# sThalham/PyraPose

Measured on AMD Instinct MI355X. Metric: images/sec 640x480 fwd+bwd (train step: fwd + losses + bwd + clipnorm-Adam), higher is better.
Workload: dtype bf16x3+f16c8

## Files before the change

include/pyrapose_hip.h:

```cpp
#ifndef PYRAPOSE_HIP_H
#define PYRAPOSE_HIP_H

#include <stddef.h>
#include <stdint.h>

#ifdef __cplusplus
extern "C" {
#endif

#define PP_OK 0
#define PP_ERR_ARG (-1)
#define PP_ERR_SHAPE (-2)
#define PP_ERR_ALIGN (-3)
#define PP_ERR_NOCTX (-4)
#define PP_ERR_UNSUPPORTED (-5)
#define PP_ERR_COMM (-6)

#define PP_MAX_SEG 5

typedef struct pp_ctx pp_ctx;

int pp_ctx_create(pp_ctx** out, int device, void* hip_stream);
void pp_ctx_destroy(pp_ctx* ctx);
int pp_ctx_set_stream(pp_ctx* ctx, void* hip_stream);
// ... 165 lines not shown
                             const int* count, float loss_weight, float* loss_sum, float* dlogits);
int pp_orth_smoothl1_fwd_bwd(pp_ctx* ctx, const pp_rowspace* rs, int n_anchor, const float* pred, int ld,
                             const float* y_true, float weight, float sigma, const int* count,
                             float loss_weight, float* loss_sum, float* dpred);

typedef struct {
  long long offset;
  long long count;
  int ld;
  int trainable;
  long long scale_off;
  float l2;
} pp_param_desc;

typedef struct pp_optimizer pp_optimizer;
int pp_optimizer_create(pp_ctx* ctx, pp_optimizer** out, const pp_param_desc* descs_host, int n_desc,
                        long long total);
void pp_optimizer_destroy(pp_optimizer* opt);
int pp_grad_global_norm(pp_ctx* ctx, pp_optimizer* opt, const float* w_master, const float* g_eff,
                        const float* scales, float* gnorm_sq, float* l2_loss);
int pp_adam_step_clipnorm(pp_ctx* ctx, pp_optimizer* opt, float* w_master, float* w_eff, const float* g_eff,
                          const float* scales, float* m, float* v, const float* gnorm_sq, float lr,
                          float beta1, float beta2, float eps, float clipnorm, long long step);

int pp_generate_base_anchors_host(int base_size, const float* ratios_host, int n_ratios,
                                  const float* scales_host, int n_scales, double* out_host);
int pp_anchors_shift_f64(pp_ctx* ctx, int n_levels, const int* feat_h_host, const int* feat_w_host,
                         const int* strides_host, int n_anchor, const double* base_anchors_host,
                         double* anchors_out);
int pp_anchors_shift_f32(pp_ctx* ctx, int n_levels, const int* feat_h_host, const int* feat_w_host,
                         const int* strides_host, int n_anchor, const double* base_anchors_host,
                         float* anchors_out);
int pp_compute_overlap_f64(pp_ctx* ctx, int n, const double* boxes, int k, const double* query, double* overlaps);
int pp_compute_gt_annotations(pp_ctx* ctx, int n, const double* anchors, int k, const double* gt_boxes,
                              double negative_overlap, double positive_overlap, int* argmax, signed char* state);

int pp_anchor_targets(pp_ctx* ctx, int n_anchor_total, const double* anchors, int batch,
                      const int* gt_offset_host, const double* gt_boxes, const int* gt_labels,
                      const double* gt_box3d, const int* gt_mask_ids, const unsigned char* id_masks,
                      int mask_h, int mask_w, const int* mask_hw_host, const int* image_hw_host, int num_classes,
                      double negative_overlap, double positive_overlap, int out_mh, int out_mw,
                      float* regression, float* labels, float* mask);
int pp_project_box3d_host(const double* pose7_host, const double* box8x3_host, const double* cam4_host,
                          double* out16_host);
int pp_pil_nearest_index_host(int n_in, int n_out, int* out_host);

// ... 196 lines not shown
```

pyrapose_amd/_lib.py:

```python
import ctypes as C
import os

_HERE = os.path.dirname(os.path.abspath(__file__))
LIB_PATH = os.path.join(_HERE, os.environ.get("PP_LIB") or "libpyrapose_hip.so")

PP_MAX_SEG = 5


class RowSpace(C.Structure):
    _fields_ = [("n_img", C.c_int), ("n_seg", C.c_int), ("h", C.c_int * PP_MAX_SEG), ("w", C.c_int * PP_MAX_SEG)]

    @classmethod
    def make(cls, n_img, shapes):
        rs = cls()
        rs.n_img = int(n_img)
        rs.n_seg = len(shapes)
        for i, (h, w) in enumerate(shapes):
            rs.h[i] = int(h)
            rs.w[i] = int(w)
        return rs

    def rows(self):
        return sum(self.n_img * self.h[i] * self.w[i] for i in range(self.n_seg))

    def shapes(self):
        return [(self.h[i], self.w[i]) for i in range(self.n_seg)]


class ConvDesc(C.Structure):
    _fields_ = [("in_", RowSpace), ("out", RowSpace), ("cin", C.c_int), ("cout", C.c_int), ("kh", C.c_int),
                ("kw", C.c_int), ("stride", C.c_int), ("pad_t", C.c_int), ("pad_l", C.c_int), ("ld_x", C.c_int),
                ("ld_y", C.c_int), ("ld_w", C.c_int)]


class ParamDesc(C.Structure):
    _fields_ = [("offset", C.c_longlong), ("count", C.c_longlong), ("ld", C.c_int), ("trainable", C.c_int),
                ("scale_off", C.c_longlong), ("l2", C.c_float)]


class SplitJob(C.Structure):
    _fields_ = [("w", C.c_void_p), ("fwd_hi", C.c_void_p), ("fwd_lo", C.c_void_p), ("dg_hi", C.c_void_p), ("dg_lo", C.c_void_p),
                ("taps", C.c_int), ("cin", C.c_int), ("cout", C.c_int), ("ld_w", C.c_int), ("tile_begin", C.c_int), ("reserved", C.c_int)]


class TView(C.Structure):
    _fields_ = [("f32", C.c_void_p), ("hi", C.c_void_p), ("lo", C.c_void_p)]


class ConvOpts(C.Structure):
    _fields_ = [("capture_hi", C.c_void_p), ("capture_lo", C.c_void_p), ("add_hi", C.c_void_p), ("add_lo", C.c_void_p),
                ("mask_hi", C.c_void_p), ("skip_flags", C.c_void_p), ("skip_list", C.c_void_p), ("out_flags", C.c_void_p),
                ("out_list", C.c_void_p), ("lazy_out", C.c_int), ("lazy_in", C.c_int)]


def _load():
    if not os.path.exists(LIB_PATH):
        raise ImportError(
            "pyrapose_amd: %s not found. Build it with `python -c 'import __graft_entry__ as g; g.build()'` "
            "or `make -C pyrapose_amd/csrc`. There is no CPU fallback." % LIB_PATH)
    try:
        return C.CDLL(LIB_PATH)
    except OSError as e:
        raise ImportError("pyrapose_amd: cannot load %s: %s" % (LIB_PATH, e))


# ... 54 lines not shown
    "pp_conv2d_nhwc_bwd_data_bf16x3": (_i, [_p, C.POINTER(ConvDesc), _p, _p, _p, _p, _p, _p, _i, _p, _i, _p, _p, _p, C.POINTER(ConvOpts)]),
    "pp_conv2d_nhwc_bwd_data_s2_bf16x3": (_i, [_p, C.POINTER(ConvDesc), _p, _p, _p, _p, _p, _p, _i, _p, _i, _p, _p, _p, C.POINTER(ConvOpts)]),
    "pp_conv_s2_merged": (_i, []),
    "pp_conv2d_nhwc_bwd_weight_bf16x3": (_i, [_p, C.POINTER(ConvDesc), _p, _p, _p, _p, _p, _p, _p, _p, C.POINTER(ConvOpts)]),
    "pp_conv_plan_text": (_i, [C.POINTER(ConvDesc), _i, C.c_uint, _i, _i, _sz, C.c_char_p, _i]),
    "pp_maxpool3x3s2_fwd": (_i, [_p, _i, _i, _i, _i, _p, _i, _i, _p]),
    "pp_upsample_nearest_add_fwd": (_i, [_p, _i, _i, _i, _i, _i, _i, _p, _p, _p]),
    "pp_upsample_nearest_add_bwd": (_i, [_p, _i, _i, _i, _i, _i, _i, _p, _p, _p]),
    "pp_add_n": (_i, [_p, _sz, _p, _p, _p, _p]),
    "pp_relu_fwd": (_i, [_p, C.c_size_t, _p, _p]),
    "pp_preprocess_caffe_u8": (_i, [_p, _i, _i, _i, C.POINTER(C.c_int), _p, _p]),
    "pp_preprocess_caffe_u8_padded": (_i, [_p, _i, _i, _i, _i, _i, _i, C.POINTER(C.c_int), _p, _p]),
    "pp_pack_rgb_to_4_padded": (_i, [_p, _i, _i, _i, _i, _i, _i, _p, _p]),
    "pp_stem7x7s2_fwd_bf16x3": (_i, [_p, _i, _i, _i, _i, _i, _p, _p, _p, _i, _p, _i, _p, _i]),
    "pp_pack_rgb_to_4": (_i, [_p, _sz, _p, _p]),
    "pp_export_head": (_i, [_p, C.POINTER(RowSpace), _i, _i, _p, _i, _i, _p]),
    "pp_count_positives": (_i, [_p, _sz, _p, _sz, _i, _p, _sz, _i, _p, _p]),
    "pp_sigmoid_focal_fwd_bwd": (_i, [_p, C.POINTER(RowSpace), _i, _i, _p, _i, _p, _f, _f, _p, _f, _p, _p]),
    "pp_orth_smoothl1_fwd_bwd": (_i, [_p, C.POINTER(RowSpace), _i, _p, _i, _p, _f, _f, _p, _f, _p, _p]),
    "pp_optimizer_create": (_i, [_p, C.POINTER(_p), C.POINTER(ParamDesc), _i, _ll]),
    "pp_optimizer_destroy": (None, [_p]),
    "pp_grad_global_norm": (_i, [_p, _p, _p, _p, _p, _p, _p]),
    "pp_adam_step_clipnorm": (_i, [_p, _p, _p, _p, _p, _p, _p, _p, _p, _f, _f, _f, _f, _f, _ll]),
    "pp_generate_base_anchors_host": (_i, [_i, C.POINTER(_f), _i, C.POINTER(_f), _i, C.POINTER(_d)]),
    "pp_anchors_shift_f64": (_i, [_p, _i, C.POINTER(_i), C.POINTER(_i), C.POINTER(_i), _i, C.POINTER(_d), _p]),
    "pp_anchors_shift_f32": (_i, [_p, _i, C.POINTER(_i), C.POINTER(_i), C.POINTER(_i), _i, C.POINTER(_d), _p]),
    "pp_compute_overlap_f64": (_i, [_p, _i, _p, _i, _p, _p]),
    "pp_compute_gt_annotations": (_i, [_p, _i, _p, _i, _p, _d, _d, _p, _p]),
    "pp_anchor_targets": (_i, [_p, _i, _p, _i, C.POINTER(_i), _p, _p, _p, _p, _p, _i, _i, C.POINTER(_i), C.POINTER(_i), _i, _d, _d,
                               _i, _i, _p, _p, _p]),
    "pp_project_box3d_host": (_i, [C.POINTER(_d), C.POINTER(_d), C.POINTER(_d), C.POINTER(_d)]),
    "pp_pil_nearest_index_host": (_i, [_i, _i, C.POINTER(_i)]),
    "pp_box3d_decode": (_i, [_p, _i, _i, _p, _p, _p]),
    "pp_score_threshold_compact": (_i, [_p, _i, _i, _i, _p, _f, _i, _p, _p]),
    "pp_filter_workspace_bytes": (_sz, [_i, _i, _i]),
    "pp_pose_error_workspace_bytes": (_sz, [_i, _i]),
    "pp_filter_detections": (_i, [_p, _i, _i, _p, _p, _p, _f, _f, _i, _p, _p, _p, _p, _p]),
    "pp_pose_add_f64": (_i, [_p, _i, _i, _p, _p, _p, _p, _p, _p, _p]),
    "pp_pose_adi_f64": (_i, [_p, _i, _i, _p, _p, _p, _p, _p, _p, _p]),
    "pp_filter_detections_batch": (_i, [_p, _i, _i, _i, _p, _p, _p, _f, _f, _i, _p, _p, _p, _p, _p]),
    "pp_render_workspace_bytes": (_sz, [_i, _i, _i, _i, _i]),
    "pp_render_depth_f32": (_i, [_p, _i, _i, _p, _i, _p, _p, _p, _p, _i, _i, _d, _d, _p, _sz, _p]),
    "pp_render_rgbd_workspace_bytes": (_sz, [_i, _i, _i, _i, _i]),
    "pp_render_rgbd": (_i, [_p, _i, _i, _p, _p, _p, _i, _p, _p, _p, _p, _i, _i, _d, _d, _i, _d, C.POINTER(_d), C.POINTER(_d), _p, _sz,
                            _p, _p, _p, _p]),
    "pp_render_rgbd_tex_workspace_bytes": (_sz, [_i, _i, _i, _i, _i, _i, _i]),
# ... 79 lines not shown
```

pyrapose_amd/csrc/conv3.hip:

```cpp
#include "conv_common.h"
#include "conv4.h"

#define PP_CAT_(a, b) a##b
#define PP_CAT(a, b) PP_CAT_(a, b)
#if PP_FMT == 1
#define PP_API(name) PP_CAT(name, _fmt1)
#else
#define PP_API(name) PP_CAT(name, _fmt0)
#endif
namespace {
#include "planes_fmt.h"

#include "conv3_shared.h"

#ifndef PP_EPI_GF
#define PP_EPI_GF 4
#endif

template <int TM, int TN, bool AP, bool OP>
__global__ __launch_bounds__(256, (TM * TN >= 8) ? 2 : ((TM * TN == 4) ? 3 : 4)) void igemm3_kernel(
    const IgemmParams p, const float* __restrict__ g_src, const uint4* __restrict__ g_ahi, const uint4* __restrict__ g_alo,
    const uint4* __restrict__ g_whi, const uint4* __restrict__ g_wlo,
    const float* __restrict__ g_bias, const float* __restrict__ g_addend, const float* __restrict__ g_mask,
    float* __restrict__ g_out, uint2* __restrict__ g_ohi, uint2* __restrict__ g_olo, int w_rows, int w_ld8) {
// ... 1047 lines not shown
  int lo = 0, hi = n_jobs - 1;
  while (lo < hi) {
    const int mid = (lo + hi + 1) >> 1;
    if (jobs[mid].tile_begin <= (int)blockIdx.x) lo = mid; else hi = mid - 1;
  }
  const pp_split_job j = jobs[lo];
  const int dg_ld = (j.cout + 31) / 32 * 32;
  const int tiles_co = dg_ld / 32, tiles_ci = j.cin / 32;
  int t = (int)blockIdx.x - j.tile_begin;
  const int co_t = t % tiles_co;
  t /= tiles_co;
  const int ci_t = t % tiles_ci, tap = t / tiles_ci;
  split_weights_tile(tap, ci_t * 32, co_t * 32, j.cin, j.cout, j.ld_w, j.w, (unsigned short*)j.fwd_hi, (unsigned short*)j.fwd_lo, j.cout,
                     (unsigned short*)j.dg_hi, (unsigned short*)j.dg_lo, dg_ld);
}

}
extern "C" int PP_API(pp_conv_split_weights_bf16x3_batch)(pp_ctx* ctx, int n_jobs, const pp_split_job* jobs_dev, int total_tiles) {
  PP_REQUIRE_CTX(ctx);
  PP_CHECK_ARG(ctx, n_jobs >= 0 && total_tiles >= 0 && (n_jobs == 0 || jobs_dev), PP_ERR_ARG, "pp_conv_split_weights_bf16x3_batch: bad arguments");
  if (n_jobs == 0 || total_tiles == 0) return PP_OK;
  hipLaunchKernelGGL(split_weights_batch_kernel, dim3((unsigned)total_tiles), dim3(32, 8), 0, ctx->stream, n_jobs, jobs_dev);
  PP_CHECK_LAUNCH(ctx, "pp_conv_split_weights_bf16x3_batch");
  return PP_OK;
}
namespace {

}
extern "C" int PP_API(pp_conv_split_weights_bf16x3)(pp_ctx* ctx, const pp_conv_desc* d, const float* w, void* fwd_hi, void* fwd_lo,
                                            void* dg_hi, void* dg_lo) {
  PP_REQUIRE_CTX(ctx);
  int rc = check_desc(ctx, d, "pp_conv_split_weights_bf16x3");
  if (rc) return rc;
  PP_CHECK_ARG(ctx, w && ((fwd_hi && fwd_lo) || (dg_hi && dg_lo)), PP_ERR_ARG, "pp_conv_split_weights_bf16x3: null tensor");
  PP_CHECK_ARG(ctx, d->cin % 32 == 0, PP_ERR_SHAPE, "pp_conv_split_weights_bf16x3: cin %d must be a multiple of 32", d->cin);
  const int taps = d->kh * d->kw;
  const int dg_ld = (d->cout + 31) / 32 * 32;
  dim3 grid((unsigned)((dg_ld + 31) / 32), (unsigned)((d->cin + 31) / 32), (unsigned)taps);
  hipLaunchKernelGGL(split_weights_kernel, grid, dim3(32, 8), 0, ctx->stream, taps, d->cin, d->cout, d->ld_w, w,
                     (unsigned short*)fwd_hi, (unsigned short*)fwd_lo, d->cout, (unsigned short*)dg_hi, (unsigned short*)dg_lo, dg_ld);
  PP_CHECK_LAUNCH(ctx, "pp_conv_split_weights_bf16x3");
  return PP_OK;
}
namespace {

__global__ void rl_dilate_kernel(const IgemmParams p, const unsigned char* __restrict__ in_flags, unsigned char* __restrict__ out_flags,
// ... 1041 lines not shown
```

pyrapose_amd/csrc/optim.hip:

```cpp
#include <math.h>
#include <stdlib.h>

#include "pp_internal.h"

#define PP_OPT_CHUNK 1024

struct pp_optimizer {
  pp_param_desc* d_descs;
  int2* d_map;
  double* d_partial;
  double* d_partial_l2;
  int n_desc;
  int n_blocks;
  long long total;
};

extern "C" int pp_optimizer_create(pp_ctx* ctx, pp_optimizer** out, const pp_param_desc* descs, int n_desc, long long total) {
  PP_REQUIRE_CTX(ctx);
  PP_CHECK_ARG(ctx, out && descs && n_desc > 0 && total > 0, PP_ERR_ARG, "pp_optimizer_create: bad argument");
  long long n_blocks = 0;
  for (int i = 0; i < n_desc; ++i) {
    PP_CHECK_ARG(ctx, descs[i].offset >= 0 && descs[i].count > 0 && descs[i].offset + descs[i].count <= total && descs[i].ld > 0 &&
                          descs[i].offset % 4 == 0,
                 PP_ERR_SHAPE, "pp_optimizer_create: tensor %d out of range", i);
    n_blocks += (descs[i].count + PP_OPT_CHUNK - 1) / PP_OPT_CHUNK;
  }
  PP_CHECK_ARG(ctx, n_blocks < (1ll << 30), PP_ERR_SHAPE, "pp_optimizer_create: too many chunks");
  pp_optimizer* o = (pp_optimizer*)calloc(1, sizeof(pp_optimizer));
  if (!o) return pp_fail(ctx, PP_ERR_ARG, "pp_optimizer_create: out of host memory");
  o->n_desc = n_desc;
  o->n_blocks = (int)n_blocks;
  o->total = total;
  int2* map = (int2*)malloc(sizeof(int2) * (size_t)n_blocks);
  long long b = 0;
  for (int i = 0; i < n_desc; ++i) {
    long long nc = (descs[i].count + PP_OPT_CHUNK - 1) / PP_OPT_CHUNK;
    for (long long c = 0; c < nc; ++c) map[b++] = make_int2(i, (int)c);
  }
  hipError_t e = hipMalloc((void**)&o->d_descs, sizeof(pp_param_desc) * n_desc);
  if (e == hipSuccess) e = hipMalloc((void**)&o->d_map, sizeof(int2) * (size_t)n_blocks);
  if (e == hipSuccess) e = hipMalloc((void**)&o->d_partial, sizeof(double) * (size_t)n_blocks);
  if (e == hipSuccess) e = hipMalloc((void**)&o->d_partial_l2, sizeof(double) * (size_t)n_blocks);
  if (e == hipSuccess) e = hipMemcpy(o->d_descs, descs, sizeof(pp_param_desc) * n_desc, hipMemcpyHostToDevice);
  if (e == hipSuccess) e = hipMemcpy(o->d_map, map, sizeof(int2) * (size_t)n_blocks, hipMemcpyHostToDevice);
  free(map);
  if (e != hipSuccess) {
    pp_optimizer_destroy(o);
    return pp_fail(ctx, (int)e, "pp_optimizer_create: %s", hipGetErrorString(e));
  }
  *out = o;
  return PP_OK;
}

extern "C" void pp_optimizer_destroy(pp_optimizer* o) {
  if (!o) return;
  if (o->d_descs) (void)hipFree(o->d_descs);
  if (o->d_map) (void)hipFree(o->d_map);
  if (o->d_partial) (void)hipFree(o->d_partial);
  if (o->d_partial_l2) (void)hipFree(o->d_partial_l2);
  free(o);
}

__device__ __forceinline__ float eff_grad(const pp_param_desc& d, long long e, const float* g_eff, const float* w_master,
                                          const float* scales) {
  float g = g_eff[d.offset + e];
  if (d.scale_off >= 0) g *= scales[d.scale_off + (e % d.ld)];
  if (d.l2 != 0.f) g += 2.0f * d.l2 * w_master[d.offset + e];
  return g;
}

__global__ void grad_norm_partial_kernel(const pp_param_desc* __restrict__ descs, const int2* __restrict__ map,
                                         const float* __restrict__ w_master, const float* __restrict__ g_eff,
                                         const float* __restrict__ scales, double* __restrict__ partial,
                                         double* __restrict__ partial_l2) {
  const int2 mp = map[blockIdx.x];
  const pp_param_desc d = descs[mp.x];
  const long long base = (long long)mp.y * PP_OPT_CHUNK;
  double s = 0.0, s2 = 0.0;
  if (d.trainable) {
#pragma unroll
    for (int k = 0; k < PP_OPT_CHUNK / 256; ++k) {
      const long long e = base + threadIdx.x + 256 * k;
      if (e < d.count) {
        const float g = eff_grad(d, e, g_eff, w_master, scales);
        s += (double)g * (double)g;
        if (d.l2 != 0.f) {
          const float w = w_master[d.offset + e];
          s2 += (double)d.l2 * (double)w * (double)w;
        }
      }
    }
// ... 33 lines not shown
    }
    __syncthreads();
  }
  if (threadIdx.x == 0) {
    gnorm_sq[0] = (float)sh[0];
    if (l2_loss) l2_loss[0] += (float)sh2[0];
  }
}

extern "C" int pp_grad_global_norm(pp_ctx* ctx, pp_optimizer* opt, const float* w_master, const float* g_eff, const float* scales,
                                   float* gnorm_sq, float* l2_loss) {
  PP_REQUIRE_CTX(ctx);
  PP_CHECK_ARG(ctx, opt && w_master && g_eff && gnorm_sq, PP_ERR_ARG, "pp_grad_global_norm: null argument");
  hipLaunchKernelGGL(grad_norm_partial_kernel, dim3((unsigned)opt->n_blocks), dim3(256), 0, ctx->stream, opt->d_descs, opt->d_map,
                     w_master, g_eff, scales, opt->d_partial, opt->d_partial_l2);
  hipLaunchKernelGGL(grad_norm_final_kernel, dim3(1), dim3(1024), 0, ctx->stream, opt->n_blocks, opt->d_partial, opt->d_partial_l2,
                     gnorm_sq, l2_loss);
  PP_CHECK_LAUNCH(ctx, "pp_grad_global_norm");
  return PP_OK;
}

__global__ void adam_kernel(const pp_param_desc* __restrict__ descs, const int2* __restrict__ map, float* __restrict__ w_master,
                            float* __restrict__ w_eff, const float* __restrict__ g_eff, const float* __restrict__ scales,
                            float* __restrict__ mom, float* __restrict__ vel, const float* __restrict__ gnorm_sq, float lr_t,
                            float beta1, float beta2, float eps, float clipnorm) {
  const int2 mp = map[blockIdx.x];
  const pp_param_desc d = descs[mp.x];
  const long long base = (long long)mp.y * PP_OPT_CHUNK;
  float clip = 1.0f;
  if (clipnorm > 0.f) {
    const float norm = sqrtf(gnorm_sq[0]);
    if (norm >= clipnorm) clip = clipnorm / norm;
  }
#pragma unroll
  for (int k = 0; k < PP_OPT_CHUNK / 256; ++k) {
    const long long e = base + threadIdx.x + 256 * k;
    if (e >= d.count) continue;
    const long long i = d.offset + e;
    float w = w_master[i];
    if (d.trainable) {
      const float g = eff_grad(d, e, g_eff, w_master, scales) * clip;
      const float m = beta1 * mom[i] + (1.0f - beta1) * g;
      const float v = beta2 * vel[i] + (1.0f - beta2) * g * g;
      mom[i] = m;
      vel[i] = v;
      w = w - lr_t * m / (sqrtf(v) + eps);
      w_master[i] = w;
    }
    w_eff[i] = d.scale_off >= 0 ? w * scales[d.scale_off + (e % d.ld)] : w;
  }
}

extern "C" int pp_adam_step_clipnorm(pp_ctx* ctx, pp_optimizer* opt, float* w_master, float* w_eff, const float* g_eff,
                                     const float* scales, float* m, float* v, const float* gnorm_sq, float lr, float beta1,
                                     float beta2, float eps, float clipnorm, long long step) {
  PP_REQUIRE_CTX(ctx);
  PP_CHECK_ARG(ctx, opt && w_master && w_eff && g_eff && m && v && gnorm_sq && step >= 1, PP_ERR_ARG,
               "pp_adam_step_clipnorm: bad argument");
  const double t = (double)step;
  const float lr_t = (float)((double)lr * sqrt(1.0 - pow((double)beta2, t)) / (1.0 - pow((double)beta1, t)));
  hipLaunchKernelGGL(adam_kernel, dim3((unsigned)opt->n_blocks), dim3(256), 0, ctx->stream, opt->d_descs, opt->d_map, w_master,
                     w_eff, g_eff, scales, m, v, gnorm_sq, lr_t, beta1, beta2, eps, clipnorm);
  PP_CHECK_LAUNCH(ctx, "pp_adam_step_clipnorm");
  return PP_OK;
}
```

pyrapose_amd/engine.py:

```python
import math
from collections import OrderedDict

import numpy as np
import torch

from . import arch, ops
from ._lib import MISSING, ParamDesc, RowSpace
from .switches import EngineSwitches


def _ru(v, m):
    return (v + m - 1) // m * m


def tf_same_pad(n_in, k, s):
    out = -(-n_in // s)
    total = max((out - 1) * s + k - n_in, 0)
    return total // 2


class Op(object):
    __slots__ = ("fn", "kind", "name", "flops", "wrange", "lane", "reads", "waits", "done_ev", "out_blocks")

    def __init__(self, fn, kind, name="", flops=0.0, wrange=None, lane=0):
# ... 185 lines not shown
        for key in self.trainable_keys():
            name, var = key.rsplit("/", 1)
            s, e = self.specs[name], self.entries[key]
            a = np.asarray(tensors[key], np.float32)
            if var == "kernel":
                if a.shape != (s.k, s.k, s.cin, s.cout):
                    raise ValueError("optimizer state of %s: shape %s, expected %s" % (key, a.shape, (s.k, s.k, s.cin, s.cout)))
                if s.cin == 3:
                    a = np.concatenate([a, np.zeros((s.k, s.k, 1, s.cout), np.float32)], axis=2)
                k2 = a.reshape(-1, s.cout)
                b = np.zeros((e["rows"], e["ld"]), np.float32)
                b[: k2.shape[0], : s.cout] = k2
                host[e["offset"]: e["offset"] + e["count"]] = b.reshape(-1)
            else:
                if a.shape != (s.cout,):
                    raise ValueError("optimizer state of %s: shape %s, expected %s" % (key, a.shape, (s.cout,)))
                host[e["offset"]: e["offset"] + s.cout] = a
        buf.copy_(torch.from_numpy(host))


class Engine(object):
    def __init__(self, ctx, num_classes, batch, height, width, backbone="resnet50", weights=None, train=True, seed=0,
                 lr=1e-5, clipnorm=0.001, freeze_backbone=False, conv_mode=None, pyramid="sparse", anchor_params=None,
                 loss_params=None):
        self.sw = sw = EngineSwitches.from_env()
        self._own_ctx = ops.Context(ctx.device, ctx.stream)
        ctx = self._own_ctx
        self.ctx, self.C, self.B, self.H, self.W = ctx, int(num_classes), int(batch), int(height), int(width)
        lp = dict(box=(0.125, 3.0), cls=(0.25, 2.0), mask=(0.25, 2.0))
        lp.update(loss_params or {})
        self.loss_params = {k: (float(v[0]), float(v[1])) for k, v in lp.items()}
        assert pyramid in arch.PYRAMIDS, pyramid
        self.pyramid = pyramid
        from .utils import anchors as _ua
        if anchor_params is None:
            anchor_params = _ua.AnchorParameters.default if pyramid != "p3p7" else _ua.AnchorParameters.p3p7
        self.anchor_params = anchor_params
        self.A = anchor_params.num_anchors()
        assert len(anchor_params.sizes) == len(arch.PYRAMID_LEVELS[pyramid]), "anchor_params need one size / stride per pyramid level"
        self.backbone = backbone
        self.train = train
        self.lr, self.clipnorm = lr, clipnorm
        self.beta1, self.beta2, self.eps = 0.9, 0.999, 1e-7
        self.specs = arch.all_specs(self.C, backbone, pyramid, self.A)
        if freeze_backbone:
            for s in self.specs:
                if s.bn:
# ... 45 lines not shown
        self.acts = OrderedDict()
        self._plane_grads = []
        self._s2_grads = []
        self.step_count = 0
        self._build_forward()
        self.levels = arch.level_shapes(self.H, self.W, arch.PYRAMID_LEVELS[pyramid])
        assert [tuple(s) for s in self.pyr.shapes] == [tuple(s) for s in self.levels], (self.pyr.shapes, self.levels)
        self.N = sum(h * w for h, w in self.levels) * self.A
        self.M3 = self.levels[0][0] * self.levels[0][1]
        f32 = dict(dtype=torch.float32, device="cuda")
        self.out_box = torch.empty((self.B, self.N, 16), **f32)
        self.out_cls = torch.empty((self.B, self.N, self.C), **f32)
        self.out_mask = torch.empty((self.B, self.M3, self.C), **f32)
        self.anchors_f32 = None
        if train:
            self.counts = torch.zeros((4,), dtype=torch.int32, device="cuda")
            self.loss_sums = torch.zeros((4,), **f32)
            self.gnorm_sq = torch.zeros((1,), **f32)
            self.y_box = torch.zeros((self.B, self.N, 17), **f32)
            self.y_cls = torch.zeros((self.B, self.N, self.C + 1), **f32)
            self.y_mask = torch.zeros((self.B, self.M3, self.C + 1), **f32)
            self.opt = ops.Optimizer(ctx, self.params.descs(), self.params.total)
            self._build_backward()
        self.grad_sync = None
        self.refresh_planes()

    def close(self):
        opt = getattr(self, "opt", None)
        if opt is not None:
            opt.close()
            self.opt = None
        st = getattr(self, "streams", None)
        if st and getattr(self, "ctxs", None):
            for side in st[1:]:
                st[0].wait_stream(side)
        for c in getattr(self, "ctxs", []):
            c.close()
        self.ctxs = []
        self.fwd_ops, self.bwd_ops, self.graph_ops = [], [], []

    def plan_signature(self):
        launches = lambda plan: [[o.kind, o.name, o.lane] for o in plan]
        return dict(fwd_ops=launches(self.fwd_ops), bwd_ops=launches(self.bwd_ops),
                    plane_grads=[list(g.shape()) + [g.fmt, bool(g.lazy), g.within is not None] for g in self._plane_grads],
                    s2_grads=[[layer, route] for layer, _, route in self._s2_grads],
                    arith=self.arith, n_lanes=self.n_lanes, prefix_lane=self.prefix_lane, switches=self.sw.non_default())

    def _enter(self):
        cur = torch.cuda.current_stream(self.ctx.device)
        if cur.cuda_stream != self.streams[0].cuda_stream:
            self.streams[0].wait_stream(cur)
        return cur

    def _leave(self, cur):
# ... 715 lines not shown
            if self.grad_sync is not None:
                self.grad_sync.reduce_counts(self.counts)
            if self.gscale is not None:
                ops.grad_scale_from_counts(ctx, self.counts[0:3], self.gscale, self.gscale_adjust)
        (bw, bs), (ca, cg), (ma, mg) = self.loss_params["box"], self.loss_params["cls"], self.loss_params["mask"]
        ops.orth_l1(ctx, self.pyr.rowspace(), self.A, self.reg_out.t, self.y_box, bw, bs, self.counts[0:1], 1.0,
                    self.loss_sums[0:1], self.g_reg)
        ops.focal(ctx, self.pyr.rowspace(), self.A, self.C, self.cls_out.t, self.y_cls, ca, cg, self.counts[1:2], 1.0,
                  self.loss_sums[1:2], self.g_cls)
        ops.focal(ctx, self.P3.rowspace(), 1, self.C, self.mask_out.t, self.y_mask, ma, mg, self.counts[2:3], 1.0,
                  self.loss_sums[2:3], self.g_mask)
        sync = self.grad_sync
        for i, op in enumerate(self.bwd_ops):
            if op.lane:
                self._fork([op.lane])
            op()
            if sync is not None:
                sync.after_bwd_op(i, self.streams[op.lane])
        self._join(list(range(1, self.n_lanes)))
        self._leave(cur)

    def refresh_planes(self, only_trainable=False):
        key = "_split_trainable" if only_trainable else "_split_all"
        if not only_trainable and getattr(self, "stem3", False):
            self._refresh_stem()
        batches = getattr(self, key, None)
        if batches is None:
            batches = []
            for fmt in (0, 1):
                jobs = [(pl["desc"], pl["w"], pl["fwd_hi"], pl["fwd_lo"], pl["dg_hi"], pl["dg_lo"]) for name, pl in self.planes.items()
                        if pl.get("fmt", 0) == fmt and (not only_trainable or self.params.specs[name].trainable)]
                if jobs:
                    batches.append((fmt, ops.SplitWeightsBatch(jobs)))
            setattr(self, key, batches)
        for fmt, batch in batches:
            batch.run(self.ctx.twin(fmt))

    def optimizer_step(self):
        P = self.params
        cur = self._enter()
        self.step_count += 1
        self.opt.grad_norm(P.w_master, P.grad, P.scales, self.gnorm_sq, self.loss_sums[3:4])
        self.opt.adam_step(P.w_master, P.w_eff, P.grad, P.scales, P.m, P.v, self.gnorm_sq, self.lr, self.beta1, self.beta2,
                           self.eps, self.clipnorm, self.step_count)
        self.refresh_planes(only_trainable=True)
        self._leave(cur)

    def train_step(self, x=None, targets=None, next_x=None):
        if targets is not None:
            self.set_targets(*targets)
        self._train_forward(lambda: self.forward(x, next_x))
        self.loss_and_backward()
        if self.grad_sync is not None:
            self.grad_sync.finish()
        self.optimizer_step()

    def _train_forward(self, run_forward):
        if not self.sparse_fwd:
            return run_forward()
        cur = self._enter()
        self._sparse_forward_lists()
        self._leave(cur)
        self._sparse_fwd_now = True
        try:
            run_forward()
        finally:
            self._sparse_fwd_now = False

    def train_step_from_annotations(self, images_u8, annotations, image_group=None, transforms=None, border="replicate", cval=0,
# ... 70 lines not shown
```

pyrapose_amd/ops.py:

```python
import collections
import ctypes as C

import numpy as np
import torch

from ._lib import ConvDesc, ConvOpts, ParamDesc, RowSpace, TView, check, lib
from ._lib import check as check_status


def _ptr(t):
    if t is None:
        return None
    assert t.is_cuda, "pyrapose_amd ops need device tensors"
    return C.c_void_p(t.data_ptr())


class Context:

    def __init__(self, device=0, stream=None):
        if not torch.cuda.is_available():
            raise RuntimeError("pyrapose_amd: no GPU visible (torch.cuda.is_available() is False); "
                               "the HIP path has no CPU fallback")
        self.device = int(device)
        torch.cuda.set_device(self.device)
# ... 438 lines not shown


class Optimizer:
    def __init__(self, ctx, descs, total):
        arr = (ParamDesc * len(descs))(*descs)
        self.handle = C.c_void_p()
        self.ctx = ctx
        check(lib.pp_optimizer_create(ctx.handle, C.byref(self.handle), arr, len(descs), total), ctx.handle,
              "pp_optimizer_create")

    def grad_norm(self, w_master, g_eff, scales, gnorm_sq, l2_loss=None):
        check(lib.pp_grad_global_norm(self.ctx.handle, self.handle, _ptr(w_master), _ptr(g_eff), _ptr(scales),
                                      _ptr(gnorm_sq), _ptr(l2_loss)), self.ctx.handle, "pp_grad_global_norm")

    def adam_step(self, w_master, w_eff, g_eff, scales, m, v, gnorm_sq, lr, beta1, beta2, eps, clipnorm, step):
        check(lib.pp_adam_step_clipnorm(self.ctx.handle, self.handle, _ptr(w_master), _ptr(w_eff), _ptr(g_eff), _ptr(scales),
                                        _ptr(m), _ptr(v), _ptr(gnorm_sq), lr, beta1, beta2, eps, clipnorm, int(step)),
              self.ctx.handle, "pp_adam_step_clipnorm")

    def close(self):
        if self.handle:
            lib.pp_optimizer_destroy(self.handle)
            self.handle = C.c_void_p()


def _iarr(v):
    return (C.c_int * len(v))(*[int(x) for x in v])


def generate_base_anchors(base_size, ratios, scales):
    r = np.ascontiguousarray(ratios, np.float32)
    s = np.ascontiguousarray(scales, np.float32)
    out = np.empty((len(r) * len(s), 4), np.float64)
    check(lib.pp_generate_base_anchors_host(int(base_size), r.ctypes.data_as(C.POINTER(C.c_float)), len(r),
                                            s.ctypes.data_as(C.POINTER(C.c_float)), len(s),
                                            out.ctypes.data_as(C.POINTER(C.c_double))), None, "pp_generate_base_anchors_host")
    return out


def anchors_shift(ctx, feat_shapes, strides, base_anchors, dtype=torch.float64):
    base = np.ascontiguousarray(base_anchors, np.float64)
    L, A = base.shape[0], base.shape[1]
    n = sum(h * w for h, w in feat_shapes) * A
    out = torch.empty((n, 4), dtype=dtype, device="cuda")
    fn = lib.pp_anchors_shift_f64 if dtype == torch.float64 else lib.pp_anchors_shift_f32
    check(fn(ctx.handle, L, _iarr([h for h, _ in feat_shapes]), _iarr([w for _, w in feat_shapes]), _iarr(strides), A,
# ... 976 lines not shown
```

Baseline: 628.4.

## Fuse Adam update with bf16x3 weight-plane splitting and widen grad-norm reduction

The conv weight tensors are now updated by a tiled Adam kernel that also encodes the new weights straight into the forward and data-grad hi/lo planes, using a shared-memory transpose. This removes the separate w_eff write and the later split pass that re-read w_eff. Non-plane parameters still go through the flat Adam kernel. The grad-norm reduction uses a wider vectorised kernel with wave-level shuffles. The cost is extra job tables and alignment constraints on the flat buffers, plus a full w_eff refresh in refresh_planes for the non-trainable path.

```diff
diff --git a/include/pyrapose_hip.h b/include/pyrapose_hip.h
--- a/include/pyrapose_hip.h
+++ b/include/pyrapose_hip.h
@@ -211,6 +211,18 @@
 int pp_adam_step_clipnorm(pp_ctx* ctx, pp_optimizer* opt, float* w_master, float* w_eff, const float* g_eff,
                           const float* scales, float* m, float* v, const float* gnorm_sq, float lr,
                           float beta1, float beta2, float eps, float clipnorm, long long step);
+typedef struct pp_adam_plane_job {
+  long long offset;
+  long long scale_off;
+  void* fwd_hi; void* fwd_lo; void* dg_hi; void* dg_lo;
+  int taps, cin, cout, ld_w;
+  int tile_begin;
+  float l2;
+} pp_adam_plane_job;
+int pp_adam_step_planes(pp_ctx* ctx, pp_optimizer* norm_opt, pp_optimizer* flat_opt, const pp_adam_plane_job* jobs_dev,
+                        int n_jobs, int total_tiles, float* w_master, float* w_eff, const float* g_eff, const float* scales,
+                        float* m, float* v, float* gnorm_sq, float* l2_loss, float lr, float beta1, float beta2, float eps,
+                        float clipnorm, long long step);
 
 int pp_generate_base_anchors_host(int base_size, const float* ratios_host, int n_ratios,
                                   const float* scales_host, int n_scales, double* out_host);
diff --git a/pyrapose_amd/_lib.py b/pyrapose_amd/_lib.py
--- a/pyrapose_amd/_lib.py
+++ b/pyrapose_amd/_lib.py
@@ -41,6 +41,12 @@
 class SplitJob(C.Structure):
     _fields_ = [("w", C.c_void_p), ("fwd_hi", C.c_void_p), ("fwd_lo", C.c_void_p), ("dg_hi", C.c_void_p), ("dg_lo", C.c_void_p),
                 ("taps", C.c_int), ("cin", C.c_int), ("cout", C.c_int), ("ld_w", C.c_int), ("tile_begin", C.c_int), ("reserved", C.c_int)]
+
+
+class AdamPlaneJob(C.Structure):
+    _fields_ = [("offset", C.c_longlong), ("scale_off", C.c_longlong), ("fwd_hi", C.c_void_p), ("fwd_lo", C.c_void_p),
+                ("dg_hi", C.c_void_p), ("dg_lo", C.c_void_p), ("taps", C.c_int), ("cin", C.c_int), ("cout", C.c_int), ("ld_w", C.c_int),
+                ("tile_begin", C.c_int), ("l2", C.c_float)]
 
 
 class TView(C.Structure):
@@ -141,6 +147,7 @@
     "pp_optimizer_destroy": (None, [_p]),
     "pp_grad_global_norm": (_i, [_p, _p, _p, _p, _p, _p, _p]),
     "pp_adam_step_clipnorm": (_i, [_p, _p, _p, _p, _p, _p, _p, _p, _p, _f, _f, _f, _f, _f, _ll]),
+    "pp_adam_step_planes": (_i, [_p, _p, _p, _p, _i, _i, _p, _p, _p, _p, _p, _p, _p, _p, _f, _f, _f, _f, _f, _ll]),
     "pp_generate_base_anchors_host": (_i, [_i, C.POINTER(_f), _i, C.POINTER(_f), _i, C.POINTER(_d)]),
     "pp_anchors_shift_f64": (_i, [_p, _i, C.POINTER(_i), C.POINTER(_i), C.POINTER(_i), _i, C.POINTER(_d), _p]),
     "pp_anchors_shift_f32": (_i, [_p, _i, C.POINTER(_i), C.POINTER(_i), C.POINTER(_i), _i, C.POINTER(_d), _p]),
diff --git a/pyrapose_amd/csrc/conv3.hip b/pyrapose_amd/csrc/conv3.hip
--- a/pyrapose_amd/csrc/conv3.hip
+++ b/pyrapose_amd/csrc/conv3.hip
@@ -1,5 +1,6 @@
 #include "conv_common.h"
 #include "conv4.h"
+#include "optim_step.h"
 
 #define PP_CAT_(a, b) a##b
 #define PP_CAT(a, b) PP_CAT_(a, b)
@@ -1093,6 +1094,85 @@
   if (n_jobs == 0 || total_tiles == 0) return PP_OK;
   hipLaunchKernelGGL(split_weights_batch_kernel, dim3((unsigned)total_tiles), dim3(32, 8), 0, ctx->stream, n_jobs, jobs_dev);
   PP_CHECK_LAUNCH(ctx, "pp_conv_split_weights_bf16x3_batch");
+  return PP_OK;
+}
+namespace {
+
+__global__ __launch_bounds__(256) void adam_planes_kernel(int n_jobs, const pp_adam_plane_job* __restrict__ jobs, float* __restrict__ w_master,
+                                                          const float* __restrict__ g_eff, const float* __restrict__ scales,
+                                                          float* __restrict__ mom, float* __restrict__ vel,
+                                                          const float* __restrict__ gnorm_sq, pp_adam_consts c) {
+  int lo = 0, hi = n_jobs - 1;
+  while (lo < hi) {
+    const int mid = (lo + hi + 1) >> 1;
+    if (jobs[mid].tile_begin <= (int)blockIdx.x) lo = mid; else hi = mid - 1;
+  }
+  const pp_adam_plane_job j = jobs[lo];
+  const int dg_ld = (j.cout + 31) / 32 * 32;
+  const int tiles_co = (j.ld_w + 31) / 32, tiles_ci = j.cin / 32;
+  int t = (int)blockIdx.x - j.tile_begin;
+  const int co0 = (t % tiles_co) * 32;
+  t /= tiles_co;
+  const int ci0 = (t % tiles_ci) * 32, tap = t / tiles_ci;
+  if (tap >= j.taps) return;
+
+  __shared__ unsigned tile[32][33];
+  const int r = threadIdx.x >> 3, q4 = (threadIdx.x & 7) * 4;
+  const float clip = pp_clip_factor(gnorm_sq, c.clipnorm);
+  const bool has_scale = j.scale_off >= 0;
+  {
+    const int ci = ci0 + r, co = co0 + q4;
+    unsigned short uh[4] = {0, 0, 0, 0}, ul[4] = {0, 0, 0, 0};
+    float enc[4] = {0.f, 0.f, 0.f, 0.f};
+    if (co < j.ld_w) {
+      const long long i = j.offset + ((long long)tap * j.cin + ci) * j.ld_w + co;
+      const float4 w4 = *reinterpret_cast<const float4*>(w_master + i), g4 = *reinterpret_cast<const float4*>(g_eff + i);
+      const float4 m4 = *reinterpret_cast<const float4*>(mom + i), v4 = *reinterpret_cast<const float4*>(vel + i);
+      float w[4] = {w4.x, w4.y, w4.z, w4.w}, m[4] = {m4.x, m4.y, m4.z, m4.w}, v[4] = {v4.x, v4.y, v4.z, v4.w};
+      const float g[4] = {g4.x, g4.y, g4.z, g4.w};
+#pragma unroll
+      for (int k = 0; k < 4; ++k) {
+        const float sc = has_scale ? scales[j.scale_off + co + k] : 1.0f;
+        w[k] = pp_adam_element(pp_eff_grad(g[k], has_scale, sc, j.l2, w[k]), clip, w[k], m[k], v[k], c);
+        if (co + k < j.cout) enc[k] = has_scale ? w[k] * sc : w[k];
+      }
+      *reinterpret_cast<float4*>(w_master + i) = make_float4(w[0], w[1], w[2], w[3]);
+      *reinterpret_cast<float4*>(mom + i) = make_float4(m[0], m[1], m[2], m[3]);
+      *reinterpret_cast<float4*>(vel + i) = make_float4(v[0], v[1], v[2], v[3]);
+    }
+#pragma unroll
+    for (int k = 0; k < 4; ++k) {
+      fmt_encode_weight(enc[k], &uh[k], &ul[k]);
+      tile[r][q4 + k] = (unsigned)uh[k] | ((unsigned)ul[k] << 16);
+    }
+    if (j.dg_hi && co < dg_ld) {
+      const long long o = ((long long)tap * j.cin + ci) * dg_ld + co;
+      *reinterpret_cast<uint2*>((unsigned short*)j.dg_hi + o) = make_uint2(uh[0] | ((unsigned)uh[1] << 16), uh[2] | ((unsigned)uh[3] << 16));
+      *reinterpret_cast<uint2*>((unsigned short*)j.dg_lo + o) = make_uint2(ul[0] | ((unsigned)ul[1] << 16), ul[2] | ((unsigned)ul[3] << 16));
+    }
+  }
+  __syncthreads();
+  if (j.fwd_hi) {
+    const int co = co0 + r, ci = ci0 + q4;
+    if (co < j.cout) {
+      const unsigned e0 = tile[q4][r], e1 = tile[q4 + 1][r], e2 = tile[q4 + 2][r], e3 = tile[q4 + 3][r];
+      const long long o = ((long long)tap * j.cout + co) * j.cin + ci;
+      *reinterpret_cast<uint2*>((unsigned short*)j.fwd_hi + o) = make_uint2((e0 & 0xffffu) | (e1 << 16), (e2 & 0xffffu) | (e3 << 16));
+      *reinterpret_cast<uint2*>((unsigned short*)j.fwd_lo + o) = make_uint2((e0 >> 16) | (e1 & 0xffff0000u), (e2 >> 16) | (e3 & 0xffff0000u));
+    }
+  }
+}
+
+}
+extern "C" int PP_API(pp_adam_planes_tiles)(pp_ctx* ctx, int n_jobs, const pp_adam_plane_job* jobs_dev, int total_tiles, float* w_master,
+                                            const float* g_eff, const float* scales, float* m, float* v, const float* gnorm_sq,
+                                            pp_adam_consts c) {
+  PP_REQUIRE_CTX(ctx);
+  PP_CHECK_ARG(ctx, n_jobs > 0 && total_tiles > 0 && jobs_dev && w_master && g_eff && m && v && gnorm_sq, PP_ERR_ARG,
+               "pp_adam_step_planes: bad tile arguments");
+  hipLaunchKernelGGL(adam_planes_kernel, dim3((unsigned)total_tiles), dim3(256), 0, ctx->stream, n_jobs, jobs_dev, w_master, g_eff, scales, m,
+                     v, gnorm_sq, c);
+  PP_CHECK_LAUNCH(ctx, "pp_adam_step_planes");
   return PP_OK;
 }
 namespace {
diff --git a/pyrapose_amd/csrc/optim.hip b/pyrapose_amd/csrc/optim.hip
--- a/pyrapose_amd/csrc/optim.hip
+++ b/pyrapose_amd/csrc/optim.hip
@@ -1,6 +1,7 @@
 #include <math.h>
 #include <stdlib.h>
 
+#include "optim_step.h"
 #include "pp_internal.h"
 
 #define PP_OPT_CHUNK 1024
@@ -13,6 +14,7 @@
   int n_desc;
   int n_blocks;
   long long total;
+  long long max_count;
 };
 
 extern "C" int pp_optimizer_create(pp_ctx* ctx, pp_optimizer** out, const pp_param_desc* descs, int n_desc, long long total) {
@@ -31,6 +33,7 @@
   o->n_desc = n_desc;
   o->n_blocks = (int)n_blocks;
   o->total = total;
+  for (int i = 0; i < n_desc; ++i) o->max_count = descs[i].count > o->max_count ? descs[i].count : o->max_count;
   int2* map = (int2*)malloc(sizeof(int2) * (size_t)n_blocks);
   long long b = 0;
   for (int i = 0; i < n_desc; ++i) {
@@ -63,10 +66,9 @@
 
 __device__ __forceinline__ float eff_grad(const pp_param_desc& d, long long e, const float* g_eff, const float* w_master,
                                           const float* scales) {
-  float g = g_eff[d.offset + e];
-  if (d.scale_off >= 0) g *= scales[d.scale_off + (e % d.ld)];
-  if (d.l2 != 0.f) g += 2.0f * d.l2 * w_master[d.offset + e];
-  return g;
+  const bool has_scale = d.scale_off >= 0;
+  return pp_eff_grad(g_eff[d.offset + e], has_scale, has_scale ? scales[d.scale_off + (e % d.ld)] : 1.0f, d.l2,
+                     d.l2 != 0.f ? w_master[d.offset + e] : 0.f);
 }
 
 __global__ void grad_norm_partial_kernel(const pp_param_desc* __restrict__ descs, const int2* __restrict__ map,
@@ -146,16 +148,11 @@
 
 __global__ void adam_kernel(const pp_param_desc* __restrict__ descs, const int2* __restrict__ map, float* __restrict__ w_master,
                             float* __restrict__ w_eff, const float* __restrict__ g_eff, const float* __restrict__ scales,
-                            float* __restrict__ mom, float* __restrict__ vel, const float* __restrict__ gnorm_sq, float lr_t,
-                            float beta1, float beta2, float eps, float clipnorm) {
+                            float* __restrict__ mom, float* __restrict__ vel, const float* __restrict__ gnorm_sq, pp_adam_consts c) {
   const int2 mp = map[blockIdx.x];
   const pp_param_desc d = descs[mp.x];
   const long long base = (long long)mp.y * PP_OPT_CHUNK;
-  float clip = 1.0f;
-  if (clipnorm > 0.f) {
-    const float norm = sqrtf(gnorm_sq[0]);
-    if (norm >= clipnorm) clip = clipnorm / norm;
-  }
+  const float clip = pp_clip_factor(gnorm_sq, c.clipnorm);
 #pragma unroll
   for (int k = 0; k < PP_OPT_CHUNK / 256; ++k) {
     const long long e = base + threadIdx.x + 256 * k;
@@ -163,16 +160,22 @@
     const long long i = d.offset + e;
     float w = w_master[i];
     if (d.trainable) {
-      const float g = eff_grad(d, e, g_eff, w_master, scales) * clip;
-      const float m = beta1 * mom[i] + (1.0f - beta1) * g;
-      const float v = beta2 * vel[i] + (1.0f - beta2) * g * g;
+      float m = mom[i], v = vel[i];
+      w = pp_adam_element(eff_grad(d, e, g_eff, w_master, scales), clip, w, m, v, c);
       mom[i] = m;
       vel[i] = v;
-      w = w - lr_t * m / (sqrtf(v) + eps);
       w_master[i] = w;
     }
     w_eff[i] = d.scale_off >= 0 ? w * scales[d.scale_off + (e % d.ld)] : w;
   }
+}
+
+static pp_adam_consts adam_consts(float lr, float beta1, float beta2, float eps, float clipnorm, long long step) {
+  const double t = (double)step;
+  pp_adam_consts c;
+  c.lr_t = (float)((double)lr * sqrt(1.0 - pow((double)beta2, t)) / (1.0 - pow((double)beta1, t)));
+  c.beta1 = beta1, c.beta2 = beta2, c.eps = eps, c.clipnorm = clipnorm;
+  return c;
 }
 
 extern "C" int pp_adam_step_clipnorm(pp_ctx* ctx, pp_optimizer* opt, float* w_master, float* w_eff, const float* g_eff,
@@ -181,10 +184,99 @@
   PP_REQUIRE_CTX(ctx);
   PP_CHECK_ARG(ctx, opt && w_master && w_eff && g_eff && m && v && gnorm_sq && step >= 1, PP_ERR_ARG,
                "pp_adam_step_clipnorm: bad argument");
-  const double t = (double)step;
-  const float lr_t = (float)((double)lr * sqrt(1.0 - pow((double)beta2, t)) / (1.0 - pow((double)beta1, t)));
   hipLaunchKernelGGL(adam_kernel, dim3((unsigned)opt->n_blocks), dim3(256), 0, ctx->stream, opt->d_descs, opt->d_map, w_master,
-                     w_eff, g_eff, scales, m, v, gnorm_sq, lr_t, beta1, beta2, eps, clipnorm);
+                     w_eff, g_eff, scales, m, v, gnorm_sq, adam_consts(lr, beta1, beta2, eps, clipnorm, step));
   PP_CHECK_LAUNCH(ctx, "pp_adam_step_clipnorm");
   return PP_OK;
 }
+
+#define PP_NORM_WAVES 4
+#define PP_NORM_CPW 4
+
+__global__ __launch_bounds__(64 * PP_NORM_WAVES) void grad_norm_wide_kernel(int n_chunks, const pp_param_desc* __restrict__ descs,
+                                                                            const int2* __restrict__ map,
+                                                                            const float* __restrict__ w_master,
+                                                                            const float* __restrict__ g_eff,
+                                                                            const float* __restrict__ scales, double* __restrict__ partial,
+                                                                            double* __restrict__ partial_l2) {
+  const int lane = threadIdx.x & 63, wave = threadIdx.x >> 6;
+  for (int k = 0; k < PP_NORM_CPW; ++k) {
+    const int chunk = ((int)blockIdx.x * PP_NORM_WAVES + wave) * PP_NORM_CPW + k;
+    if (chunk >= n_chunks) return;
+    const int2 mp = map[chunk];
+    const pp_param_desc d = descs[mp.x];
+    const bool has_scale = d.scale_off >= 0;
+    const unsigned count = (unsigned)d.count, ld = (unsigned)d.ld;
+    double s = 0.0, s2 = 0.0;
+    if (d.trainable) {
+#pragma unroll
+      for (int q = 0; q < PP_OPT_CHUNK / 256; ++q) {
+        const unsigned e = (unsigned)mp.y * PP_OPT_CHUNK + 256u * q + 4u * lane;
+        if (e >= count) continue;
+        float g[4] = {0.f, 0.f, 0.f, 0.f}, w[4] = {0.f, 0.f, 0.f, 0.f};
+        const int n = count - e < 4u ? (int)(count - e) : 4;
+        if (n == 4) {
+          const float4 g4 = *reinterpret_cast<const float4*>(g_eff + d.offset + e);
+          g[0] = g4.x, g[1] = g4.y, g[2] = g4.z, g[3] = g4.w;
+          if (d.l2 != 0.f) {
+            const float4 w4 = *reinterpret_cast<const float4*>(w_master + d.offset + e);
+            w[0] = w4.x, w[1] = w4.y, w[2] = w4.z, w[3] = w4.w;
+          }
+        } else {
+          for (int t = 0; t < n; ++t) {
+            g[t] = g_eff[d.offset + e + t];
+            if (d.l2 != 0.f) w[t] = w_master[d.offset + e + t];
+          }
+        }
+        unsigned col = has_scale ? e % ld : 0u;
+#pragma unroll
+        for (int t = 0; t < 4; ++t) {
+          if (t < n) {
+            const float ge = pp_eff_grad(g[t], has_scale, has_scale ? scales[d.scale_off + col] : 1.0f, d.l2, w[t]);
+            s += (double)ge * (double)ge;
+            if (d.l2 != 0.f) s2 += (double)d.l2 * (double)w[t] * (double)w[t];
+          }
+          if (++col >= ld) col = 0u;
+        }
+      }
+    }
+#pragma unroll
+    for (int o = 32; o > 0; o >>= 1) {
+      s += __shfl_xor(s, o, 64);
+      s2 += __shfl_xor(s2, o, 64);
+    }
+    if (lane == 0) {
+      partial[chunk] = s;
+      partial_l2[chunk] = s2;
+    }
+  }
+}
+
+extern "C" int pp_adam_step_planes(pp_ctx* ctx, pp_optimizer* norm_opt, pp_optimizer* flat_opt, const pp_adam_plane_job* jobs_dev,
+                                   int n_jobs, int total_tiles, float* w_master, float* w_eff, const float* g_eff, const float* scales,
+                                   float* m, float* v, float* gnorm_sq, float* l2_loss, float lr, float beta1, float beta2, float eps,
+                                   float clipnorm, long long step) {
+  PP_REQUIRE_CTX(ctx);
+  PP_CHECK_ARG(ctx, w_master && g_eff && m && v && gnorm_sq && step >= 1 && n_jobs >= 0 && total_tiles >= 0 && (n_jobs == 0 || jobs_dev) &&
+                        (!flat_opt || w_eff),
+               PP_ERR_ARG, "pp_adam_step_planes: bad argument");
+  PP_CHECK_ARG(ctx, pp_is_aligned16(w_master) && pp_is_aligned16(g_eff) && pp_is_aligned16(m) && pp_is_aligned16(v), PP_ERR_ALIGN,
+               "pp_adam_step_planes: the flat buffers must be 16-byte aligned");
+  PP_CHECK_ARG(ctx, !norm_opt || norm_opt->max_count < (1ll << 31), PP_ERR_SHAPE, "pp_adam_step_planes: a tensor of 2^31 elements or more");
+  const pp_adam_consts c = adam_consts(lr, beta1, beta2, eps, clipnorm, step);
+  if (norm_opt) {
+    const int per_wg = PP_NORM_WAVES * PP_NORM_CPW;
+    hipLaunchKernelGGL(grad_norm_wide_kernel, dim3((unsigned)((norm_opt->n_blocks + per_wg - 1) / per_wg)), dim3(64 * PP_NORM_WAVES), 0,
+                       ctx->stream, norm_opt->n_blocks, norm_opt->d_descs, norm_opt->d_map, w_master, g_eff, scales, norm_opt->d_partial,
+                       norm_opt->d_partial_l2);
+    hipLaunchKernelGGL(grad_norm_final_kernel, dim3(1), dim3(1024), 0, ctx->stream, norm_opt->n_blocks, norm_opt->d_partial,
+                       norm_opt->d_partial_l2, gnorm_sq, l2_loss);
+  }
+  if (flat_opt)
+    hipLaunchKernelGGL(adam_kernel, dim3((unsigned)flat_opt->n_blocks), dim3(256), 0, ctx->stream, flat_opt->d_descs, flat_opt->d_map,
+                       w_master, w_eff, g_eff, scales, m, v, gnorm_sq, c);
+  PP_CHECK_LAUNCH(ctx, "pp_adam_step_planes");
+  if (n_jobs == 0 || total_tiles == 0) return PP_OK;
+  return ctx->planes_fmt == 1 ? pp_adam_planes_tiles_fmt1(ctx, n_jobs, jobs_dev, total_tiles, w_master, g_eff, scales, m, v, gnorm_sq, c)
+                              : pp_adam_planes_tiles_fmt0(ctx, n_jobs, jobs_dev, total_tiles, w_master, g_eff, scales, m, v, gnorm_sq, c);
+}
diff --git a/pyrapose_amd/csrc/optim_step.h b/pyrapose_amd/csrc/optim_step.h
--- /dev/null
+++ b/pyrapose_amd/csrc/optim_step.h
@@ -0,0 +1,39 @@
+#pragma once
+#include <hip/hip_runtime.h>
+
+#include "pp_internal.h"
+
+struct pp_adam_consts {
+  float lr_t, beta1, beta2, eps, clipnorm;
+};
+
+__device__ __forceinline__ float pp_clip_factor(const float* __restrict__ gnorm_sq, float clipnorm) {
+  float clip = 1.0f;
+  if (clipnorm > 0.f) {
+    const float norm = sqrtf(gnorm_sq[0]);
+    if (norm >= clipnorm) clip = clipnorm / norm;
+  }
+  return clip;
+}
+
+__device__ __forceinline__ float pp_eff_grad(float g, bool has_scale, float scale, float l2, float w) {
+#pragma clang fp contract(off)
+  if (has_scale) g *= scale;
+  if (l2 != 0.f) g = fmaf(2.0f * l2, w, g);
+  return g;
+}
+
+__device__ __forceinline__ float pp_adam_element(float g_eff, float clip, float w, float& m, float& v, const pp_adam_consts& c) {
+#pragma clang fp contract(off)
+  const float g = g_eff * clip;
+  m = c.beta1 * m + (1.0f - c.beta1) * g;
+  v = c.beta2 * v + (1.0f - c.beta2) * g * g;
+  return w - c.lr_t * m / (sqrtf(v) + c.eps);
+}
+
+extern "C" int pp_adam_planes_tiles_fmt0(pp_ctx* ctx, int n_jobs, const pp_adam_plane_job* jobs_dev, int total_tiles, float* w_master,
+                                         const float* g_eff, const float* scales, float* m, float* v, const float* gnorm_sq,
+                                         pp_adam_consts c);
+extern "C" int pp_adam_planes_tiles_fmt1(pp_ctx* ctx, int n_jobs, const pp_adam_plane_job* jobs_dev, int total_tiles, float* w_master,
+                                         const float* g_eff, const float* scales, float* m, float* v, const float* gnorm_sq,
+                                         pp_adam_consts c);
diff --git a/pyrapose_amd/engine.py b/pyrapose_amd/engine.py
--- a/pyrapose_amd/engine.py
+++ b/pyrapose_amd/engine.py
@@ -231,7 +231,7 @@
 class Engine(object):
     def __init__(self, ctx, num_classes, batch, height, width, backbone="resnet50", weights=None, train=True, seed=0,
                  lr=1e-5, clipnorm=0.001, freeze_backbone=False, conv_mode=None, pyramid="sparse", anchor_params=None,
-                 loss_params=None):
+                 loss_params=None, fused_opt=True):
         self.sw = sw = EngineSwitches.from_env()
         self._own_ctx = ops.Context(ctx.device, ctx.stream)
         ctx = self._own_ctx
@@ -323,6 +323,8 @@
             self.y_mask = torch.zeros((self.B, self.M3, self.C + 1), **f32)
             self.opt = ops.Optimizer(ctx, self.params.descs(), self.params.total)
             self._build_backward()
+        self.fused_opt = bool(fused_opt) and train and self.conv_mode == "bf16x3"
+        self._fused = None
         self.grad_sync = None
         self.refresh_planes()
 
@@ -331,6 +333,10 @@
         if opt is not None:
             opt.close()
             self.opt = None
+        for o in (getattr(self, "_fused", None) or (None, None))[:2]:
+            if o is not None:
+                o.close()
+        self._fused = None
         st = getattr(self, "streams", None)
         if st and getattr(self, "ctxs", None):
             for side in st[1:]:
@@ -1092,6 +1098,8 @@
 
     def refresh_planes(self, only_trainable=False):
         key = "_split_trainable" if only_trainable else "_split_all"
+        if not only_trainable and self.conv_mode == "bf16x3":
+            self.params.refresh_eff()
         if not only_trainable and getattr(self, "stem3", False):
             self._refresh_stem()
         batches = getattr(self, key, None)
@@ -1110,11 +1118,43 @@
         P = self.params
         cur = self._enter()
         self.step_count += 1
-        self.opt.grad_norm(P.w_master, P.grad, P.scales, self.gnorm_sq, self.loss_sums[3:4])
-        self.opt.adam_step(P.w_master, P.w_eff, P.grad, P.scales, P.m, P.v, self.gnorm_sq, self.lr, self.beta1, self.beta2,
-                           self.eps, self.clipnorm, self.step_count)
-        self.refresh_planes(only_trainable=True)
+        if self.fused_opt:
+            norm_opt, flat_opt, batches = self._fused or self._fused_tables()
+            for i, (fmt, jobs) in enumerate(batches):
+                ops.adam_step_planes(self.ctx.twin(fmt), norm_opt if i == 0 else None, flat_opt if i == 0 else None, jobs, P.w_master,
+                                     P.w_eff, P.grad, P.scales, P.m, P.v, self.gnorm_sq, self.loss_sums[3:4] if i == 0 else None,
+                                     self.lr, self.beta1, self.beta2, self.eps, self.clipnorm, self.step_count)
+        else:
+            self.opt.grad_norm(P.w_master, P.grad, P.scales, self.gnorm_sq, self.loss_sums[3:4])
+            self.opt.adam_step(P.w_master, P.w_eff, P.grad, P.scales, P.m, P.v, self.gnorm_sq, self.lr, self.beta1, self.beta2,
+                               self.eps, self.clipnorm, self.step_count)
+            self.refresh_planes(only_trainable=True)
         self._leave(cur)
+
+    def _fused_tables(self):
+        P = self.params
+        descs = dict(zip(P.entries, P.descs()))
+        owners = OrderedDict((name + "/kernel", pl) for name, pl in self.planes.items() if P.specs[name].trainable)
+        train = [d for key, d in descs.items() if P.entries[key]["trainable"]]
+        flat = [d for key, d in descs.items() if P.entries[key]["trainable"] and key not in owners]
+        norm_opt = ops.Optimizer(self.ctx, train, P.total) if train else None
+        flat_opt = ops.Optimizer(self.ctx, flat, P.total) if flat else None
+        batches = []
+        for fmt in (0, 1):
+            jobs = []
+            for key, pl in owners.items():
+                if pl.get("fmt", 0) != fmt:
+                    continue
+                e, d = P.entries[key], pl["desc"]
+                assert d.ld_w == e["ld"] and d.kh * d.kw * d.cin * d.ld_w == e["count"], key
+                jobs.append((e["offset"], e["scale_off"], e["l2"], d.kh * d.kw, d.cin, d.cout, d.ld_w, pl["fwd_hi"], pl["fwd_lo"],
+                             pl["dg_hi"], pl["dg_lo"]))
+            if jobs:
+                batches.append((fmt, ops.AdamPlaneJobs(jobs)))
+        if not batches:
+            batches = [(0, None)]
+        self._fused = (norm_opt, flat_opt, batches)
+        return self._fused
 
     def train_step(self, x=None, targets=None, next_x=None):
         if targets is not None:
diff --git a/pyrapose_amd/ops.py b/pyrapose_amd/ops.py
--- a/pyrapose_amd/ops.py
+++ b/pyrapose_amd/ops.py
@@ -484,6 +484,47 @@
         if self.handle:
             lib.pp_optimizer_destroy(self.handle)
             self.handle = C.c_void_p()
+
+
+class AdamPlaneJobs(object):
+
+    def __init__(self, jobs):
+        from ._lib import AdamPlaneJob
+        jobs = list(jobs)
+        arr = (AdamPlaneJob * max(len(jobs), 1))()
+        tiles = 0
+        self._keep = jobs
+        for i, (off, soff, l2, taps, cin, cout, ld_w, fh, fl, dh, dl) in enumerate(jobs):
+            if cin % 32 or ld_w % 4 or off % 4 or cout > ld_w:
+                raise ValueError("AdamPlaneJobs: cin %d %% 32, ld_w %d %% 4, offset %d %% 4 must be 0 and cout %d <= ld_w" % (cin, ld_w, off, cout))
+            for t, shape in ((fh, (taps, cout, cin)), (fl, (taps, cout, cin)), (dh, (taps, cin, (cout + 31) // 32 * 32)),
+                             (dl, (taps, cin, (cout + 31) // 32 * 32))):
+                if t is not None and (tuple(t.shape) != shape or not t.is_contiguous() or t.element_size() != 2):
+                    raise ValueError("AdamPlaneJobs: a plane of shape %s where %s is expected" % (tuple(t.shape), shape))
+            if (fh is None) != (fl is None) or (dh is None) != (dl is None):
+                raise ValueError("AdamPlaneJobs: hi and lo planes go together")
+            j = arr[i]
+            j.fwd_hi, j.fwd_lo, j.dg_hi, j.dg_lo = [(t.data_ptr() if t is not None else None) for t in (fh, fl, dh, dl)]
+            j.offset, j.scale_off, j.l2 = int(off), int(soff), float(l2)
+            j.taps, j.cin, j.cout, j.ld_w, j.tile_begin = taps, cin, cout, ld_w, tiles
+            tiles += taps * (cin // 32) * ((ld_w + 31) // 32)
+        self.n, self.tiles = len(jobs), tiles
+        self.extent = max([off + taps * cin * ld_w for off, _, _, taps, cin, _, ld_w, _, _, _, _ in jobs] or [0])
+        self.scale_extent = max([soff + ld_w for _, soff, _, _, _, _, ld_w, _, _, _, _ in jobs if soff >= 0] or [0])
+        host = torch.frombuffer(bytearray(bytes(arr)), dtype=torch.uint8)
+        self.table = host.cuda()
+
+
+def adam_step_planes(ctx, norm_opt, flat_opt, jobs, w_master, w_eff, g_eff, scales, m, v, gnorm_sq, l2_loss, lr, beta1, beta2, eps,
+                     clipnorm, step):
+    n, tiles, table = (jobs.n, jobs.tiles, jobs.table) if jobs is not None else (0, 0, None)
+    if jobs is not None and jobs.extent > min(t.numel() for t in (w_master, g_eff, m, v)):
+        raise ValueError("adam_step_planes: a job reaches past the end of the flat buffers")
+    if jobs is not None and jobs.scale_extent > (scales.numel() if scales is not None else 0):
+        raise ValueError("adam_step_planes: a job reaches past the end of the scales")
+    check(lib.pp_adam_step_planes(ctx.handle, norm_opt.handle if norm_opt is not None else None, flat_opt.handle if flat_opt is not None else None,
+                                  _ptr(table), n, tiles, _ptr(w_master), _ptr(w_eff), _ptr(g_eff), _ptr(scales), _ptr(m), _ptr(v),
+                                  _ptr(gnorm_sq), _ptr(l2_loss), lr, beta1, beta2, eps, clipnorm, int(step)), ctx.handle, "pp_adam_step_planes")
 
 
 def _iarr(v):
```

Result: no change. 632.6, median of 6 (+0.7%).
